# ALRhub/d3il

Measured on AMD Instinct MI355X. Metric: env-steps/s, higher is better.
Workload: dtype f64

## Files before the change

### d3il_amd/capi.py

```python
from __future__ import annotations

import ctypes as C
import os

from .model.blob import ModelBlob

_LIB = None


class Buffers(C.Structure):
    _fields_ = [("n_envs", C.c_int32), ("stride", C.c_int32), ("obs_dim", C.c_int32), ("action_dim", C.c_int32),
                ("obs", C.c_void_p), ("done", C.c_void_p), ("success", C.c_void_p), ("mode", C.c_void_p),
                ("state", C.c_void_p), ("flags", C.c_void_p), ("step_count", C.c_void_p), ("policy_des", C.c_void_p),
                ("info_f64", C.c_void_p), ("n_info_f64", C.c_int32), ("state_rows", C.c_int32), ("last_reset", C.c_void_p)]


STATE_F64 = 42
STATE_QPOS, STATE_QVEL, STATE_BIAS, STATE_TCP, STATE_IK_Q, STATE_IK_QD = 0, 9, 18, 25, 28, 35
FLAG_MODE_MASK, FLAG_TERMINATED, FLAG_SUCCESS, FLAG_ROD_CONTACT = 0x1FF, 1 << 12, 1 << 13, 1 << 14
FLAG_IK_VALID, FLAG_SOLVER_FAIL, FLAG_MULTI_CONTACT = 1 << 15, 1 << 16, 1 << 17
PUSH_STATE_BOX, PUSH_STATE_WARM, PUSH_STATE_TASK, PUSH_STATE_F64 = 42, 68, 89, 91
PFLAG_FIRST_MASK, PFLAG_MODE_MASK, PFLAG_WARM_VALID, PFLAG_CON_OVERFLOW, PFLAG_OFF_TABLE = 0x7, 0x38, 1 << 6, 1 << 18, 1 << 19
PFLAG_LINK_NEAR = 1 << 20
LINK_GUARD_SLACK = 1.25e-4
# ... 28 lines not shown
    if os.environ.get("D3IL_LIB_PATH"):
        return os.environ["D3IL_LIB_PATH"]
    name = "libd3il_rollout_stats.so" if os.environ.get("D3IL_STATS_LIB") == "1" else "libd3il_rollout.so"
    return os.path.join(os.path.dirname(os.path.abspath(__file__)), name)


def load():
    global _LIB
    if _LIB is None:
        path = lib_path()
        if not os.path.exists(path):
            raise D3ilError("%s is missing: build it with `python -m d3il_amd.build` (hipcc, gfx950). "
                            "There is no CPU fallback for the rollout path." % path)
        L = C.CDLL(path)
        L.d3il_last_error.restype = C.c_char_p
        L.d3il_blob_sizeof.restype = C.c_size_t
        L.d3il_create.argtypes = [C.c_int, C.c_int, C.c_int, C.c_void_p, C.c_size_t, C.POINTER(C.c_void_p)]
        L.d3il_destroy.argtypes = [C.c_void_p]
        L.d3il_start.argtypes = [C.c_void_p, C.c_void_p]
        L.d3il_reset.argtypes = [C.c_void_p, C.c_void_p, C.c_void_p, C.c_void_p]
        L.d3il_step.argtypes = [C.c_void_p, C.c_void_p, C.c_void_p]
        L.d3il_get_buffers.argtypes = [C.c_void_p, C.POINTER(Buffers)]
        L.d3il_get_state.argtypes = [C.c_void_p, C.c_void_p, C.c_int32, C.c_void_p, C.c_void_p]
        L.d3il_set_state.argtypes = [C.c_void_p, C.c_void_p, C.c_int32, C.c_void_p, C.c_void_p]
        L.d3il_policy_begin.argtypes = [C.c_void_p, C.c_void_p, C.c_void_p]
        L.d3il_policy_action.argtypes = [C.c_void_p, C.c_uint64, C.c_uint64, C.c_uint32, C.c_void_p, C.c_void_p]
        L.d3il_count_metrics.argtypes = [C.c_void_p, C.c_void_p, C.c_void_p]
        L.d3il_attention_causal_f32.argtypes = [C.c_void_p, C.c_void_p, C.c_int, C.c_int, C.c_int, C.c_int, C.c_void_p]
        L.d3il_layernorm_f32.argtypes = [C.c_void_p, C.c_void_p, C.c_void_p, C.c_void_p, C.c_long, C.c_int, C.c_float, C.c_void_p]
        L.d3il_mlp_ln_gelu_residual_f32.argtypes = [C.c_void_p, C.c_void_p, C.c_void_p, C.c_float, C.c_void_p, C.c_void_p, C.c_void_p, C.c_void_p, C.c_void_p, C.c_long, C.c_int, C.c_int, C.c_void_p]
        L.d3il_linear120_f32.argtypes = [C.c_void_p, C.c_void_p, C.c_void_p, C.c_float, C.c_void_p, C.c_void_p, C.c_void_p, C.c_void_p, C.c_long, C.c_int, C.c_void_p]
        L.d3il_mlp_ln_gelu_residual_f16x3.argtypes = L.d3il_mlp_ln_gelu_residual_f32.argtypes
        L.d3il_linear120_f16x3.argtypes = L.d3il_linear120_f32.argtypes
        L.d3il_attn_half_f16x3.argtypes = [C.c_void_p, C.c_void_p, C.c_void_p, C.c_float, C.c_void_p, C.c_void_p, C.c_void_p, C.c_void_p, C.c_long, C.c_int, C.c_int, C.c_int, C.c_void_p]
        L.d3il_f16x3_set_guard.argtypes = [C.c_void_p]
        L.d3il_bet_head_f32.argtypes = [C.c_void_p, C.c_void_p, C.c_void_p, C.c_float] + [C.c_void_p] * 6 + [C.c_uint64, C.c_uint64] + [C.c_void_p] * 6 + [C.c_long, C.c_int, C.c_int, C.c_int, C.c_void_p]
        L.d3il_ddpm_gpt_step_f32.argtypes = [C.c_void_p, C.c_void_p, C.c_void_p, C.c_float] + [C.c_void_p] * 11 + [C.c_uint64, C.c_uint64] + [C.c_void_p] * 7 + [C.c_long] + [C.c_int] * 5 + [C.c_void_p]
        L.d3il_ibc_langevin_f32.argtypes = [C.c_void_p] * 10 + [C.c_float] + [C.c_void_p] * 5 + [C.c_uint64, C.c_uint64] + [C.c_void_p] * 11 + [C.c_long] + [C.c_int] * 6 + [C.c_void_p]
        L.d3il_act_chunk_f32.argtypes = [C.c_void_p] * 12 + [C.c_uint64, C.c_uint64] + [C.c_void_p] * 6 + [C.c_long] + [C.c_int] * 8 + [C.c_void_p]
        L.d3il_ddpm_act_chunk_f32.argtypes = [C.c_void_p] * 13 + [C.c_uint64, C.c_uint64] + [C.c_void_p] * 9 + [C.c_long] + [C.c_int] * 12 + [C.c_void_p]
        L.d3il_cvae_decode_f32.argtypes = [C.c_void_p] * 11 + [C.c_uint64, C.c_uint64] + [C.c_void_p] * 4 + [C.c_long] + [C.c_int] * 5 + [C.c_void_p]
        L.d3il_ddpm_mlp_f32.argtypes = [C.c_void_p] * 12 + [C.c_long, C.c_int, C.c_int, C.c_int, C.c_int, C.c_void_p]
        L.d3il_resmlp_f32.argtypes = [C.c_void_p] * 8 + [C.c_long, C.c_int, C.c_int, C.c_int, C.c_int, C.c_void_p]
        L.d3il_mlp_gelu_residual_f32.argtypes = [C.c_void_p, C.c_void_p, C.c_void_p, C.c_void_p, C.c_void_p, C.c_void_p, C.c_long, C.c_int, C.c_int, C.c_void_p]
        L.d3il_auto_reset.argtypes = [C.c_void_p, C.c_void_p, C.c_void_p]
        L.d3il_step_auto_reset.argtypes = [C.c_void_p, C.c_void_p, C.c_void_p, C.c_void_p]
        L.d3il_random_rollout_step.argtypes = [C.c_void_p, C.c_uint64, C.c_uint64, C.c_uint32, C.c_void_p, C.c_void_p, C.c_void_p]
        L.d3il_random_rollout_prepare.argtypes = [C.c_void_p, C.c_uint64, C.c_uint64, C.c_uint32, C.c_void_p, C.c_void_p, C.c_void_p]
        L.d3il_timing_stats.argtypes = [C.c_void_p, C.c_void_p]
        L.d3il_set_tally.argtypes = [C.c_void_p, C.c_void_p, C.c_int, C.c_void_p]
        L.d3il_comm_unique_id.argtypes = [C.c_void_p]
        L.d3il_comm_init.argtypes = [C.c_void_p, C.c_int, C.c_int, C.c_int, C.POINTER(C.c_void_p)]
        L.d3il_comm_destroy.argtypes = [C.c_void_p]
        L.d3il_comm_count.argtypes = [C.c_void_p, C.POINTER(C.c_int)]
        L.d3il_rccl_available.restype = C.c_int
        L.d3il_reduce_metrics.argtypes = [C.c_void_p, C.c_void_p, C.c_void_p, C.c_size_t, C.c_void_p]
        L.d3il_set_timing.argtypes = [C.c_void_p, C.c_int]
        L.d3il_last_step_ms.argtypes = [C.c_void_p, C.POINTER(C.c_float)]
        L.d3il_set_option.argtypes = [C.c_void_p, C.c_char_p, C.c_int]
        L.d3il_debug_scratch.argtypes = [C.c_void_p, C.c_int, C.c_void_p, C.c_int]
        L.d3il_debug_build_flags.argtypes = [C.c_void_p]
        L.d3il_set_link_guard.argtypes = [C.c_void_p, C.c_void_p, C.c_int, C.c_double, C.c_void_p]
        if hasattr(L, "d3il_group_create"):
            L.d3il_group_create.argtypes = [C.c_void_p, C.c_int, C.POINTER(C.c_void_p)]
            L.d3il_group_flush.argtypes = [C.c_void_p]
            L.d3il_group_destroy.argtypes = [C.c_void_p]
        if hasattr(L, "d3il_group_set_option"):
            L.d3il_group_set_option.argtypes = [C.c_void_p, C.c_char_p, C.c_int]
            L.d3il_group_stats.argtypes = [C.c_void_p, C.POINTER(C.c_int64), C.POINTER(C.c_int64)]
        if L.d3il_blob_sizeof() != C.sizeof(ModelBlob):
            raise D3ilError("model blob layout mismatch between include/d3il_model_blob.h and d3il_amd/model/blob.py")
        _LIB = L
    return _LIB


def has_step_group() -> bool:
    return hasattr(load(), "d3il_group_create")


def has_group_options() -> bool:
    return hasattr(load(), "d3il_group_set_option")


def check(rc: int):
    if rc != 0:
        raise D3ilError("libd3il_rollout error %d: %s" % (rc, load().d3il_last_error().decode()))


_CAPSULES = os.path.join(os.path.dirname(os.path.abspath(__file__)), "model", "blobs", "panda_link_capsules.json")


def link_capsules(body_names, path: str | None = None):
    import json
    import numpy as np
    with open(path or _CAPSULES) as f:
        js = json.load(f)
    rows = [[body_names.index(c["body"]), c["statics"]] + list(c["p0"]) + list(c["p1"]) + [c["r"]] for c in js["capsules"]]
    return np.ascontiguousarray(rows, dtype=np.float64), float(js["margin"])


def set_link_guard(h, capsules, margin: float, counter_ptr=None):
    import numpy as np
    caps = np.zeros((0, 9)) if capsules is None else np.ascontiguousarray(capsules, dtype=np.float64).reshape(-1, 9)
    check(load().d3il_set_link_guard(h, caps.ctypes.data_as(C.c_void_p) if len(caps) else None, len(caps), float(margin), counter_ptr))
```

### d3il_amd/csrc/rollout.hip

```cpp
#include <hip/hip_runtime.h>
#include <cstdio>
#include <cstdlib>
#include <cstring>
#include <dlfcn.h>
#include <memory>
#include <mutex>
#include <string>
#include "../../include/d3il_rollout.h"
#include "panda_step.h"
#include "rigid_common.h"
#include "gen/avoiding_consts.inc"
#include "gen/stacking_consts.inc"

namespace d3il {
constexpr int WAVE = 64;
}
#include "gen_kernels.h"
#include "link_guard.h"
#include "stack_kernels.h"
#include "policy_f16x3.h"
#include "policy_bet.h"
#include "policy_ddpm_gpt.h"
#include "policy_ibc.h"
#include "policy_act.h"
// ... 871 lines not shown
  if (episode_counts) {
    atomicAdd((unsigned long long*)&episode_counts[0], 1ull);
    if (success[e]) atomicAdd((unsigned long long*)&episode_counts[1], 1ull);
  }
  if (!table) return;
  int c = ctx_id ? ctx_id[e] : 0;
  if (c < 0 || c >= n_ctx) return;
  long long* row = table + (size_t)c * D3IL_TALLY_ROW;
  atomicAdd((unsigned long long*)&row[0], 1ull);
  int code = (int)(short)mode[e] + mode_bias;
  if (success[e]) {
    atomicAdd((unsigned long long*)&row[1], 1ull);
    if (code >= 0 && code < D3IL_TALLY_ROW - 2) atomicAdd((unsigned long long*)&row[2 + code], 1ull);
  }
  if (all_by_code && code >= 0 && code < 256) atomicAdd((unsigned long long*)&row[2 + D3IL_TALLY_ALL + code], 1ull);
}
__global__ void k_store_contexts(const unsigned char* __restrict__ mask, const double* __restrict__ src, double* __restrict__ dst, int n, int dim) {
  int i = blockIdx.x * blockDim.x + threadIdx.x;
  if (i >= n * dim) return;
  if (mask && !mask[i / dim]) return;
  dst[i] = src[i];
}

}

using namespace d3il;

static_assert(D3IL_STACK_STATE_BOX == SK_STATE_BOX && D3IL_STACK_STATE_WARM == SK_STATE_WARM && D3IL_STACK_STATE_F64 == SK_STATE_F64, "d3il_rollout.h: Stacking state layout");
static_assert(D3IL_SFLAG_WARM_VALID == SKF_WARM_VALID && D3IL_SFLAG_HAND_NEAR == SKF_HAND_NEAR && D3IL_PFLAG_CON_OVERFLOW == SKF_CON_OVERFLOW && D3IL_PFLAG_OFF_TABLE == SKF_OFF_TABLE,
              "d3il_rollout.h: Stacking flag bits");
static_assert(D3IL_PFLAG_LINK_NEAR == LG_FLAG && D3IL_PFLAG_LINK_NEAR == D3IL_SFLAG_HAND_NEAR, "d3il_rollout.h: the link-near bit of the generic engine is the hand-near bit of the cooperative one");
static_assert(D3IL_SFLAG_MODE_MASK == (SKF_NMODE_MASK | (0x3Fu << SKF_IND_SHIFT)), "d3il_rollout.h: Stacking order code");
static_assert(D3IL_ALIGN_STATE_BOX == AL_STATE_BOX && D3IL_ALIGN_STATE_WARM == AL_STATE_WARM && D3IL_ALIGN_STATE_TARGET == AL_STATE_TARGET && D3IL_ALIGN_STATE_F64 == AL_STATE_F64, "d3il_rollout.h: Aligning state layout");
static_assert(D3IL_INS_STATE_BOX == 42 && D3IL_INS_STATE_WARM == 42 + 13 * 3 && D3IL_INS_STATE_TASK == 42 + 13 * 3 + 6 * 3 + NDOF && D3IL_INS_STATE_F64 == gen_state_rows(3), "d3il_rollout.h: Inserting state layout");
static_assert(D3IL_PUSH_STATE_BOX == 42 && D3IL_PUSH_STATE_WARM == 42 + 13 * 2 && D3IL_PUSH_STATE_TASK == 42 + 13 * 2 + 6 * 2 + NDOF && D3IL_PUSH_STATE_F64 == gen_state_rows(2) && D3IL_TALLY_ALL + 256 <= D3IL_TALLY_ROW - 2,
              "d3il_rollout.h: Pushing state rows / tally row");

static inline bool gen_task(int task_id) {
  return task_id == D3IL_TASK_SORTING || task_id == D3IL_TASK_INSERTING || task_id == D3IL_TASK_PUSHING;
}

constexpr int RG_SLOTS = 2, RG_SAMPLE = 8;
struct d3il_handle_s {
  int task_id, n, stride, device;
  PandaConsts hc;
  PandaConsts* dc;
  GenConsts gc;
  StackConsts kc;
  AlignTask atk;
  double* d_scratch;
  int state_rows;
  double* d_init_qpos;
  bool started;
  d3il_buffers buf;
  bool fast, timing;
  int split;
  bool serve_avail;
  int serve_max_wg;
  int lanes;
  int lds_pad;
  hipEvent_t ev0, ev1;
  bool ev_valid, ev_created;
  hipEvent_t ring0[128], ring1[128];
  bool ring_created;
  long ring_head, ring_drained, t_n;
  double t_sum, t_min, t_max;
  int tol_mode;
  int stack_reset_coop;
  unsigned long long kc_id;
  double* d_ctx;
  int ctx_dim;
  uint8_t* d_mask;
  const int32_t* tally_ctx; int tally_nctx; int64_t* tally_table;
  bool rg_enabled, rg_ready, rg_capturing, rg_ev_made, rg_timing;
  int rg_slot;
  hipGraph_t rg_graph[RG_SLOTS]; hipGraphExec_t rg_exec[RG_SLOTS];
  unsigned* rg_t_dev; uint32_t rg_next_t; long rg_launched, rg_drained;
  uint64_t rg_seed, rg_off; double* rg_actions; int64_t* rg_counts; hipStream_t rg_stream;
  void* d_reset_img; AvoidResetImage reset_img; AvoidEpilogue* d_epilogue; AvoidEpilogue epilogue_host; bool epilogue_valid; hipStream_t epilogue_stream;
  bool prep_valid; uint32_t prep_t; uint64_t prep_seed, prep_off; double* prep_actions; bool fuse_tail; double* d_des_before; hipStream_t prep_stream;
  bool info_is_view;
  d3il_model_blob model;
  LinkGuardConsts lg; LinkGuardConsts* d_lg; int64_t* lg_flagged;
  struct d3il_group_s* group; bool grp_pending; uint64_t grp_seed, grp_off; uint32_t grp_t; double* grp_actions; int64_t* grp_counts; hipStream_t grp_stream;
  hipEvent_t ring_alt0[128], ring_alt1[128];
};
struct d3il_group_s {
  int device, count; d3il_handle_s* m[AVOID_GROUP_MAX];
  int n_pending; bool busy;
  uint32_t t; int n_substeps, max_steps; bool timing;
  AvoidGroupTable* d_table; AvoidGroupTable table_host; bool table_valid;
  hipEvent_t ev_join[AVOID_GROUP_MAX], ev_done; bool ev_made;
  hipEvent_t ring0[128], ring1[128]; bool ring_created; long ring_head;
  bool quiet, armed; int64_t n_merged, n_joined;
};
static inline void group_arm(d3il_group_s* g) { g->armed = true; }
#if defined(D3IL_EVENT_SYSTEM_FENCE)
constexpr unsigned EV_ORDER_FLAGS = hipEventDisableTiming, EV_TIMING_FLAGS = hipEventDefault;
#else
constexpr unsigned EV_ORDER_FLAGS = hipEventDisableTiming | hipEventDisableSystemFence, EV_TIMING_FLAGS = hipEventDefault | hipEventDisableSystemFence;
#endif

struct ActiveModel { int refs; bool valid; GenConsts gc; StackConsts kc; };
static ActiveModel g_active_gen[16], g_active_stack[16];
static int g_active_tol[16];
static std::mutex g_model_mutex;

static unsigned long long g_stack_loaded_id[16];
static StackConsts g_stack_loaded[16];
static unsigned long long g_kc_counter = 0;

static thread_local std::string g_err;
static int fail(int code, const std::string& msg) { g_err = msg; return code; }
#define HIPCHK(x) do { hipError_t e_ = (x); if (e_ != hipSuccess) return fail(D3IL_EHIP, std::string(#x) + ": " + hipGetErrorString(e_)); } while (0)

extern "C" {

static int group_flush(d3il_group_s* g);
static inline int group_settle(d3il_handle_s* h) {
  if (!h || !h->group || h->group->busy) return D3IL_OK;
  group_arm(h->group);
  return h->group->n_pending ? group_flush(h->group) : D3IL_OK;
}
#define GROUP_SETTLE(h) do { if (int rc_g_ = group_settle(h)) return rc_g_; } while (0)

const char* d3il_last_error(void) { return g_err.c_str(); }
size_t d3il_blob_sizeof(void) { return sizeof(d3il_model_blob); }
int d3il_version(void) { return 2; }

static void rg_drop(d3il_handle_s* h);
static void group_leave(d3il_handle_s* h);
static void rg_drop_for_free(d3il_handle_s* h) {
  if (h->rg_ready) for (int k = 0; k < RG_SLOTS; k++) { (void)hipGraphExecDestroy(h->rg_exec[k]); (void)hipGraphDestroy(h->rg_graph[k]); }
  if (h->rg_t_dev) (void)hipFree(h->rg_t_dev);
}
static void free_handle(d3il_handle_s* h) {
  if (!h) return;
  int dev = h->device;
  if (dev >= 0 && dev < 16) {
    std::lock_guard<std::mutex> lock(g_model_mutex);
    if (gen_task(h->task_id) && g_active_gen[dev].refs > 0) g_active_gen[dev].refs--;
    if (h->task_id == D3IL_TASK_STACKING && g_active_stack[dev].refs > 0) g_active_stack[dev].refs--;
  }
  void* ptrs[] = {h->dc, h->d_init_qpos, h->buf.obs, h->buf.done, h->buf.success, h->buf.mode, h->buf.state, h->buf.flags, h->buf.step_count, h->buf.policy_des,
                  h->info_is_view ? nullptr : (void*)h->buf.info_f64, h->d_scratch, h->d_ctx, h->d_mask, h->d_des_before, h->d_lg, h->d_reset_img, h->d_epilogue};
  for (void* p : ptrs) if (p) (void)hipFree(p);
  if (h->ring_created) for (int i = 0; i < 128; i++) { (void)hipEventDestroy(h->ring0[i]); (void)hipEventDestroy(h->ring1[i]); }
  rg_drop_for_free(h);
  delete h;
}
#define HIPCHK_H(x) do { hipError_t e_ = (x); if (e_ != hipSuccess) { free_handle(h); return fail(D3IL_EHIP, std::string(#x) + ": " + hipGetErrorString(e_)); } } while (0)

int d3il_create(int task_id, int n_envs, int device_id, const void* model_blob, size_t blob_len, d3il_handle* out) {
  if (!out || !model_blob) return fail(D3IL_EINVAL, "d3il_create: null argument");
  *out = nullptr;
  if (blob_len != sizeof(d3il_model_blob)) return fail(D3IL_EBLOB, "d3il_create: blob size mismatch");
  if (n_envs <= 0) return fail(D3IL_EINVAL, "d3il_create: n_envs must be positive");
  const d3il_model_blob& m = *(const d3il_model_blob*)model_blob;
  if (task_id != m.task_id) return fail(D3IL_EINVAL, "d3il_create: task_id does not match the model blob");
  if (task_id != D3IL_TASK_AVOIDING && task_id != D3IL_TASK_PUSHING && task_id != D3IL_TASK_SORTING && task_id != D3IL_TASK_STACKING && task_id != D3IL_TASK_ALIGNING && task_id != D3IL_TASK_INSERTING)
    return fail(D3IL_EUNSUPPORTED, "d3il_create: unknown task id (Avoiding, Pushing, Sorting, Stacking, Aligning and Inserting are implemented)");
  int ndev = 0;
  if (hipGetDeviceCount(&ndev) != hipSuccess || ndev <= 0) return fail(D3IL_ENODEVICE, "d3il_create: no HIP device available (there is no CPU fallback)");
  if (device_id < 0 || device_id >= ndev || device_id >= 16) return fail(D3IL_ENODEVICE, "d3il_create: device_id out of range");
  HIPCHK(hipSetDevice(device_id));
  d3il_handle_s* h = new d3il_handle_s();
  std::memset(&h->buf, 0, sizeof h->buf);
  h->task_id = -1; h->device = device_id;
  h->model = m; h->d_lg = nullptr; h->lg_flagged = nullptr; h->lg.n = 0;
  h->dc = nullptr; h->d_init_qpos = nullptr; h->d_scratch = nullptr; h->d_ctx = nullptr; h->d_mask = nullptr; h->ev_created = false; h->ring_created = false;
  h->tally_ctx = nullptr; h->tally_nctx = 0; h->tally_table = nullptr; h->tol_mode = 0; h->ctx_dim = 0; h->stack_reset_coop = 1; h->kc_id = 0;
  const char* err = "";
  int rc = build_panda_consts(m, h->hc, &err);
  if (rc) { free_handle(h); return fail(D3IL_EBLOB, std::string("d3il_create: ") + err); }
  finish_invweights(h->hc);
  if (gen_task(task_id) && build_gen_consts(m, h->hc, h->gc, &err)) { free_handle(h); return fail(D3IL_EBLOB, std::string("d3il_create: ") + err); }
  if (task_id == D3IL_TASK_STACKING && build_stack_consts(m, h->hc, h->kc, &err)) { free_handle(h); return fail(D3IL_EBLOB, std::string("d3il_create: ") + err); }
  if (task_id == D3IL_TASK_ALIGNING && build_coop_align_consts(m, h->hc, h->kc, h->atk, &err)) { free_handle(h); return fail(D3IL_EBLOB, std::string("d3il_create: ") + err); }
  {
// ... 862 lines not shown
  if (!(h->rg_enabled && h->task_id == D3IL_TASK_AVOIDING && stream != nullptr && h->started)) return D3IL_OK;
  hipStream_t s = (hipStream_t)stream;
  HIPCHK(hipSetDevice(h->device));
  if (h->rg_ready && (h->rg_seed != seed || h->rg_off != env_offset || h->rg_actions != actions || h->rg_counts != episode_counts_device || h->rg_stream != s ||
                      h->rg_timing != h->timing)) {
    HIPCHK(hipStreamSynchronize(h->rg_stream));
    rg_drop(h);
  }
  if (!h->rg_ready) return rg_capture(h, seed, env_offset, t, actions, episode_counts_device, s);
  return D3IL_OK;
}
static bool continues_sequence(const d3il_handle_s* h, uint64_t seed, uint64_t env_offset, uint32_t t, const double* actions, void* stream) {
  return h->prep_valid && h->prep_t == t && h->prep_seed == seed && h->prep_off == env_offset && h->prep_actions == actions && h->prep_stream == (hipStream_t)stream;
}
static int fused_step_begin(d3il_handle h, uint64_t seed, uint64_t env_offset, uint32_t t, double* actions, int64_t* episode_counts_device, void* stream, AvoidEpilogue& a) {
  const bool cont = continues_sequence(h, seed, env_offset, t, actions, stream);
  if (!h->d_des_before) { HIPCHK(hipSetDevice(h->device)); HIPCHK(hipMalloc(&h->d_des_before, (size_t)h->stride * 2 * sizeof(double))); }
  if (cont) h->prep_valid = 0;
  else { if (int rc = d3il_policy_action(h, seed, env_offset, t, actions, stream)) return rc; }
  d3il_buffers& b = h->buf;
  a = AvoidEpilogue{};
  a.img = h->reset_img; a.state = b.state; a.flags = b.flags; a.steps = b.step_count; a.obs = b.obs; a.done = b.done; a.success = b.success; a.mode = b.mode;
  a.n = h->n; a.stride = h->stride; a.des = b.policy_des; a.episode_counts = (long long*)episode_counts_device; a.mask = h->d_mask; a.ctx_id = h->tally_ctx;
  a.table = (long long*)h->tally_table; a.actions = actions; a.des_before = h->d_des_before; a.seed = seed; a.env_offset = env_offset; a.n_ctx = h->tally_nctx;
  if (split_step_kernel(h)) {
    if (!h->epilogue_valid || std::memcmp(&h->epilogue_host, &a, sizeof a) != 0) {
      HIPCHK(hipSetDevice(h->device));
      if (h->epilogue_valid && (h->epilogue_stream != (hipStream_t)stream || h->group)) HIPCHK(hipDeviceSynchronize());
      HIPCHK(hipMemcpyAsync(h->d_epilogue, &a, sizeof a, hipMemcpyHostToDevice, (hipStream_t)stream));
      HIPCHK(hipStreamSynchronize((hipStream_t)stream));
      h->epilogue_host = a; h->epilogue_valid = true; h->epilogue_stream = (hipStream_t)stream;
    }
  }
  return D3IL_OK;
}
static void fused_step_end(d3il_handle h, uint64_t seed, uint64_t env_offset, uint32_t t, double* actions, void* stream) {
  h->prep_valid = true; h->prep_t = t + 1u; h->prep_seed = seed; h->prep_off = env_offset; h->prep_actions = actions; h->prep_stream = (hipStream_t)stream;
}
static int rollout_step_single(d3il_handle h, uint64_t seed, uint64_t env_offset, uint32_t t, double* actions, int64_t* episode_counts_device, void* stream) {
  if (h && h->rg_enabled && h->task_id == D3IL_TASK_AVOIDING && stream != nullptr && actions && h->started) {
    hipStream_t s = (hipStream_t)stream;
    if (int rc_ = drop_prepared_action(h)) return rc_;
    if (int rc = d3il_random_rollout_prepare(h, seed, env_offset, t, actions, episode_counts_device, stream)) return rc;
    if (t != h->rg_next_t) { HIPCHK(hipMemcpyAsync(h->rg_t_dev, &t, sizeof(unsigned), hipMemcpyHostToDevice, s)); HIPCHK(hipStreamSynchronize(s)); }
    if (h->timing && h->rg_launched % RG_SAMPLE == RG_SAMPLE - 1) {
      if (int rc = d3il_policy_action(h, seed, env_offset, t, actions, stream)) return rc;
      if (int rc = d3il_step(h, actions, stream)) return rc;
      if (int rc = d3il_auto_reset(h, episode_counts_device, stream)) return rc;
      hipLaunchKernelGGL(k_inc_counter, dim3(1), dim3(64), 0, s, h->rg_t_dev);
      HIPCHK(hipGetLastError());
    } else HIPCHK(hipGraphLaunch(h->rg_exec[h->rg_launched % RG_SLOTS], s));
    h->rg_launched++; h->rg_next_t = t + 1;
    return D3IL_OK;
  }
  if (h && h->fuse_tail && h->task_id == D3IL_TASK_AVOIDING && actions && episode_counts_device && h->started) {
    AvoidEpilogue a;
    if (int rc = fused_step_begin(h, seed, env_offset, t, actions, episode_counts_device, stream, a)) return rc;
    if (split_step_kernel(h)) {
      if (int rc = step_launch(h, actions, stream, h->d_epilogue, t + 1u)) return rc;
    } else {
      if (int rc = d3il_step(h, actions, stream)) return rc;
      hipLaunchKernelGGL(k_avoiding_tail, dim3(h->stride / WAVE), dim3(WAVE), 0, (hipStream_t)stream, a, t + 1u);
      HIPCHK(hipGetLastError());
    }
    fused_step_end(h, seed, env_offset, t, actions, stream);
    return D3IL_OK;
  }
  if (int rc = d3il_policy_action(h, seed, env_offset, t, actions, stream)) return rc;
  if (int rc = d3il_step(h, actions, stream)) return rc;
  return d3il_auto_reset(h, episode_counts_device, stream);
}

static int group_flush(d3il_group_s* g) {
  if (g->busy) return D3IL_OK;
  group_arm(g);
  g->busy = true;
  int rc = D3IL_OK;
  for (int i = 0; i < g->count; i++) {
    d3il_handle_s* h = g->m[i];
    if (!h->grp_pending) continue;
    h->grp_pending = false; g->n_pending--;
    if (!rc) rc = rollout_step_single(h, h->grp_seed, h->grp_off, h->grp_t, h->grp_actions, h->grp_counts, (void*)h->grp_stream);
  }
  g->n_pending = 0; g->busy = false;
  return rc;
}
static int group_launch_locked(d3il_group_s* g) {
  HIPCHK(hipSetDevice(g->device));
  if (!g->ev_made) {
    for (int i = 0; i < AVOID_GROUP_MAX; i++) HIPCHK(hipEventCreateWithFlags(&g->ev_join[i], EV_ORDER_FLAGS));
    HIPCHK(hipEventCreateWithFlags(&g->ev_done, EV_ORDER_FLAGS));
    HIPCHK(hipMalloc(&g->d_table, sizeof(AvoidGroupTable)));
    g->ev_made = true;
  }
  AvoidGroupTable tab;
  std::memset(&tab, 0, sizeof tab);
  unsigned total = 0; int serve_budget = 0;
  for (int i = 0; i < AVOID_GROUP_MAX; i++) tab.m[i].first_wg = 0xFFFFFFFFu;
  for (int i = 0; i < g->count; i++) {
    d3il_handle_s* h = g->m[i];
    AvoidEpilogue a;
    if (int rc = fused_step_begin(h, h->grp_seed, h->grp_off, h->grp_t, h->grp_actions, h->grp_counts, (void*)h->grp_stream, a)) return rc;
    const d3il_buffers& b = h->buf;
    AvoidGroupMember& r = tab.m[i];
    r.state = b.state; r.flags = b.flags; r.steps = b.step_count; r.actions = h->grp_actions; r.obs = b.obs; r.done = b.done; r.success = b.success; r.mode = b.mode;
    r.ep = h->d_epilogue; r.n = h->n; r.stride = h->stride; r.first_wg = total;
    total += (unsigned)((h->n + WAVE - 1) / WAVE); serve_budget += h->serve_max_wg;
  }
  hipStream_t s0 = g->m[0]->grp_stream;
  if (!g->table_valid || std::memcmp(&g->table_host, &tab, sizeof tab) != 0) {
    if (g->table_valid) HIPCHK(hipDeviceSynchronize());
    HIPCHK(hipMemcpy(g->d_table, &tab, sizeof tab, hipMemcpyHostToDevice));
    g->table_host = tab; g->table_valid = true;
  }
  const bool join = !g->quiet || g->armed;
  if (join) for (int i = 1; i < g->count; i++) {
    if (g->m[i]->grp_stream == s0) continue;
    HIPCHK(hipEventRecord(g->ev_join[i], g->m[i]->grp_stream));
    HIPCHK(hipStreamWaitEvent(s0, g->ev_join[i], 0));
  }
  hipEvent_t t0 = nullptr, t1 = nullptr;
  if (g->timing) {
    if (!g->ring_created) {
      for (int i = 0; i < 128; i++) { HIPCHK(hipEventCreateWithFlags(&g->ring0[i], EV_TIMING_FLAGS)); HIPCHK(hipEventCreateWithFlags(&g->ring1[i], EV_TIMING_FLAGS)); }
      g->ring_created = true;
    }
    for (int i = 0; i < g->count; i++) { d3il_handle_s* h = g->m[i]; if (h->ring_head - h->ring_drained >= 128) { if (int rc = timing_drain_one(h)) return rc; } }
    t0 = g->ring0[g->ring_head % 128]; t1 = g->ring1[g->ring_head % 128];
    HIPCHK(hipEventRecord(t0, s0));
  }
  const d3il_handle_s* h0 = g->m[0];
  const unsigned t_next = g->t + 1u;
  if ((long)total <= (long)serve_budget)
    hipLaunchKernelGGL((k_avoiding_step_split<true, true, true>), dim3(total), dim3(3 * WAVE), AVOID_LDS_SERVE, s0, (const AvoidGroupTable*)g->d_table, (double*)nullptr, (unsigned*)nullptr,
                       (int*)nullptr, (const double*)nullptr, (float*)nullptr, (unsigned char*)nullptr, (unsigned char*)nullptr, (unsigned short*)nullptr, 0, 0, h0->hc.n_substeps,
                       h0->hc.max_steps, (const AvoidEpilogue*)nullptr, t_next);
  else
    hipLaunchKernelGGL((k_avoiding_step_split<true, false, true>), dim3(total), dim3(2 * WAVE), 0, s0, (const AvoidGroupTable*)g->d_table, (double*)nullptr, (unsigned*)nullptr,
                       (int*)nullptr, (const double*)nullptr, (float*)nullptr, (unsigned char*)nullptr, (unsigned char*)nullptr, (unsigned short*)nullptr, 0, 0, h0->hc.n_substeps,
                       h0->hc.max_steps, (const AvoidEpilogue*)nullptr, t_next);
  HIPCHK(hipGetLastError());
  hipEvent_t done_ev = g->ev_done;
  if (g->timing) {
    HIPCHK(hipEventRecord(t1, s0));
    done_ev = t1;
    for (int i = 0; i < g->count; i++) {
      d3il_handle_s* h = g->m[i];
      const int slot = (int)(h->ring_head % 128);
      h->ring_alt0[slot] = t0; h->ring_alt1[slot] = t1; h->ev0 = t0; h->ev1 = t1; h->ev_valid = true; h->ring_head++;
    }
    g->ring_head++;
  } else HIPCHK(hipEventRecord(done_ev, s0));
  for (int i = 1; i < g->count; i++) if (g->m[i]->grp_stream != s0) HIPCHK(hipStreamWaitEvent(g->m[i]->grp_stream, done_ev, 0));
  for (int i = 0; i < g->count; i++) { d3il_handle_s* h = g->m[i]; fused_step_end(h, h->grp_seed, h->grp_off, h->grp_t, h->grp_actions, (void*)h->grp_stream); }
  g->n_merged++; g->n_joined += join ? 1 : 0;
  g->armed = false;
  return D3IL_OK;
}
static int group_launch(d3il_group_s* g) {
  g->busy = true;
  const int rc = group_launch_locked(g);
  if (rc) group_arm(g);
  for (int i = 0; i < g->count; i++) g->m[i]->grp_pending = false;
  g->n_pending = 0; g->busy = false;
  return rc;
}
static int group_rollout_step(d3il_handle h, uint64_t seed, uint64_t env_offset, uint32_t t, double* actions, int64_t* episode_counts_device, void* stream, int* handled) {
  d3il_group_s* g = h->group;
  *handled = 0;
  if (g->busy) return D3IL_OK;
  const bool eligible = h->fuse_tail && !h->rg_enabled && h->task_id == D3IL_TASK_AVOIDING && actions && episode_counts_device && h->started && split_step_kernel(h) &&
                        h->serve_avail && continues_sequence(h, seed, env_offset, t, actions, stream);
  if (!eligible) {
    group_arm(g);
    return g->n_pending ? group_flush(g) : D3IL_OK;
  }
  if (g->n_pending && (h->grp_pending || g->t != t || g->n_substeps != h->hc.n_substeps || g->max_steps != h->hc.max_steps || g->timing != h->timing)) {
    if (int rc = group_flush(g)) return rc;
  }
  if (!g->n_pending) { g->t = t; g->n_substeps = h->hc.n_substeps; g->max_steps = h->hc.max_steps; g->timing = h->timing; }
  h->grp_pending = true; h->grp_seed = seed; h->grp_off = env_offset; h->grp_t = t; h->grp_actions = actions; h->grp_counts = episode_counts_device; h->grp_stream = (hipStream_t)stream;
  g->n_pending++;
  *handled = 1;
  return g->n_pending == g->count ? group_launch(g) : D3IL_OK;
}
int d3il_random_rollout_step(d3il_handle h, uint64_t seed, uint64_t env_offset, uint32_t t, double* actions, int64_t* episode_counts_device, void* stream) {
  if (h && h->group) {
    int handled = 0;
    if (int rc = group_rollout_step(h, seed, env_offset, t, actions, episode_counts_device, stream, &handled)) return rc;
    if (handled) return D3IL_OK;
  }
  return rollout_step_single(h, seed, env_offset, t, actions, episode_counts_device, stream);
}
static void timing_drain_all(d3il_handle_s* h) { while (h->ring_drained < h->ring_head) { if (timing_drain_one(h)) { h->ring_drained = h->ring_head; break; } } }
static void group_leave(d3il_handle_s* h) {
  d3il_group_s* g = h->group;
  if (!g) return;
  (void)group_flush(g);
  group_arm(g);
  timing_drain_all(h);
  if (h->ring_head > 0 && h->ring_alt0[(h->ring_head - 1) % 128]) { h->ev_valid = false; h->ev0 = h->ev1 = nullptr; }
  for (int i = 0; i < 128; i++) h->ring_alt0[i] = h->ring_alt1[i] = nullptr;
  int k = 0;
  for (int i = 0; i < g->count; i++) if (g->m[i] != h) g->m[k++] = g->m[i];
  g->count = k; h->group = nullptr; h->grp_pending = false;
}
int d3il_group_create(const d3il_handle* handles, int count, d3il_group* out) {
  if (!handles || !out) return fail(D3IL_EINVAL, "d3il_group_create: null argument");
  *out = nullptr;
  if (count < 1 || count > AVOID_GROUP_MAX) return fail(D3IL_EINVAL, "d3il_group_create: a group has 1 .. 8 members");
  for (int i = 0; i < count; i++) {
    d3il_handle_s* h = handles[i];
    if (!h) return fail(D3IL_EINVAL, "d3il_group_create: null handle");
    if (h->task_id != D3IL_TASK_AVOIDING) return fail(D3IL_EUNSUPPORTED, "d3il_group_create: Avoiding handles only");
    if (h->device != handles[0]->device) return fail(D3IL_EINVAL, "d3il_group_create: the members must live on one device");
    if (h->group) return fail(D3IL_ESTATE, "d3il_group_create: a handle is already in a group");
    for (int j = 0; j < i; j++) if (handles[j] == h) return fail(D3IL_EINVAL, "d3il_group_create: a handle is listed twice");
  }
  HIPCHK(hipSetDevice(handles[0]->device));
  if (hipFuncSetAttribute((const void*)k_avoiding_step_split<true, true, true>, hipFuncAttributeMaxDynamicSharedMemorySize, (int)AVOID_LDS_SERVE) != hipSuccess) (void)hipGetLastError();
  d3il_group_s* g = new d3il_group_s();
  g->device = handles[0]->device; g->count = count;
  g->armed = true;
  for (int i = 0; i < count; i++) { g->m[i] = handles[i]; handles[i]->group = g; handles[i]->grp_pending = false; }
  *out = g;
  return D3IL_OK;
}
int d3il_group_flush(d3il_group g) {
  if (!g) return fail(D3IL_EINVAL, "d3il_group_flush: null group");
  group_arm(g);
  return g->n_pending ? group_flush(g) : D3IL_OK;
}
int d3il_group_set_option(d3il_group g, const char* name, int value) {
  if (!g || !name) return fail(D3IL_EINVAL, "d3il_group_set_option: null argument");
  if (std::strcmp(name, "quiet_streams") == 0) {
    if (value != 0 && value != 1) return fail(D3IL_EINVAL, "quiet_streams must be 0 or 1");
    group_arm(g);
    if (g->n_pending) { if (int rc = group_flush(g)) return rc; }
    g->quiet = value != 0;
    return D3IL_OK;
  }
  return fail(D3IL_EINVAL, std::string("d3il_group_set_option: unknown option ") + name);
}
int d3il_group_stats(d3il_group g, int64_t* merged_rounds, int64_t* joined_rounds) {
  if (!g || !merged_rounds || !joined_rounds) return fail(D3IL_EINVAL, "d3il_group_stats: null argument");
  *merged_rounds = g->n_merged; *joined_rounds = g->n_joined;
  return D3IL_OK;
}
int d3il_group_destroy(d3il_group g) {
  if (!g) return fail(D3IL_EINVAL, "d3il_group_destroy: null group");
  (void)hipSetDevice(g->device);
  const int rc = group_flush(g);
  while (g->count > 0) group_leave(g->m[g->count - 1]);
  (void)hipDeviceSynchronize();
  if (g->ev_made) { for (int i = 0; i < AVOID_GROUP_MAX; i++) (void)hipEventDestroy(g->ev_join[i]); (void)hipEventDestroy(g->ev_done); (void)hipFree(g->d_table); }
  if (g->ring_created) for (int i = 0; i < 128; i++) { (void)hipEventDestroy(g->ring0[i]); (void)hipEventDestroy(g->ring1[i]); }
  delete g;
  return rc;
}
int d3il_last_step_ms(d3il_handle h, float* ms) {
  GROUP_SETTLE(h);
  if (!h || !ms) return fail(D3IL_EINVAL, "d3il_last_step_ms: null argument");
  if (!h->ev_valid) return fail(D3IL_ESTATE, "d3il_last_step_ms: timing not enabled or no step recorded");
  HIPCHK(hipEventSynchronize(h->ev1));
  HIPCHK(hipEventElapsedTime(ms, h->ev0, h->ev1));
  return D3IL_OK;
}
int d3il_debug_wave_stats(uint64_t* out, int nwaves, int reset) {
#if defined(D3IL_DEVICE_STATS)
  HIPCHK(hipDeviceSynchronize());
  HIPCHK(hipMemcpyFromSymbol(out, HIP_SYMBOL(d3il::g_dev_wave), (size_t)nwaves * 10 * sizeof(unsigned long long)));
  if (reset) { static unsigned long long z[4096][10]; HIPCHK(hipMemcpyToSymbol(HIP_SYMBOL(d3il::g_dev_wave), z, sizeof z)); }
  return D3IL_OK;
#else
  (void)out; (void)nwaves; (void)reset;
  return fail(D3IL_EUNSUPPORTED, "d3il_debug_wave_stats: library built without D3IL_DEVICE_STATS");
#endif
}

int d3il_debug_wave_counts(uint64_t* out, int nwaves, int reset) {
#if defined(D3IL_DEVICE_STATS)
  HIPCHK(hipDeviceSynchronize());
  HIPCHK(hipMemcpyFromSymbol(out, HIP_SYMBOL(d3il::g_dev_cnt), (size_t)nwaves * 8 * sizeof(unsigned long long)));
  if (reset) { static unsigned long long z[4096][8]; HIPCHK(hipMemcpyToSymbol(HIP_SYMBOL(d3il::g_dev_cnt), z, sizeof z)); }
  return D3IL_OK;
#else
  (void)out; (void)nwaves; (void)reset;
  return fail(D3IL_EUNSUPPORTED, "d3il_debug_wave_counts: library built without D3IL_DEVICE_STATS");
#endif
}

int d3il_debug_stats(uint64_t* out32, int reset) {
#if defined(D3IL_DEVICE_STATS)
  unsigned long long tmp[32];
  HIPCHK(hipDeviceSynchronize());
  HIPCHK(hipMemcpyFromSymbol(tmp, HIP_SYMBOL(d3il::g_dev_stats), sizeof tmp));
  for (int i = 0; i < 32; i++) out32[i] = tmp[i];
  if (reset) { unsigned long long z[32] = {0}; HIPCHK(hipMemcpyToSymbol(HIP_SYMBOL(d3il::g_dev_stats), z, sizeof z)); }
  return D3IL_OK;
#else
  (void)out32; (void)reset;
  return fail(D3IL_EUNSUPPORTED, "d3il_debug_stats: library built without D3IL_DEVICE_STATS");
#endif
}

int d3il_debug_scratch(d3il_handle h, int env, double* out, int count) {
  GROUP_SETTLE(h);
  if (!h || !out) return fail(D3IL_EINVAL, "d3il_debug_scratch: null argument");
  if (!h->d_scratch || env < 0 || env >= h->n) return fail(D3IL_EINVAL, "d3il_debug_scratch: no scratch area / env out of range");
  HIPCHK(hipSetDevice(h->device));
  HIPCHK(hipDeviceSynchronize());
  if (h->task_id == D3IL_TASK_STACKING || h->task_id == D3IL_TASK_ALIGNING) {
    if (count > SG_SIZE) return fail(D3IL_EINVAL, "d3il_debug_scratch: count exceeds the environment's scratch area");
    HIPCHK(hipMemcpy(out, h->d_scratch + (size_t)env * SG_SIZE, (size_t)count * sizeof(double), hipMemcpyDeviceToHost));
    return D3IL_OK;
  }
  if (gen_task(h->task_id)) {
    if (count > GG_SIZE) return fail(D3IL_EINVAL, "d3il_debug_scratch: count exceeds the environment's scratch area");
    const double* base = h->d_scratch + (size_t)(env / GEN_LANES) * GG_BLOCK * GEN_LANES + 2 * (env % GEN_LANES);
    HIPCHK(hipMemcpy2D(out, 2 * sizeof(double), base, (size_t)2 * GEN_LANES * sizeof(double), sizeof(double), (size_t)(count + 1) / 2, hipMemcpyDeviceToHost));
    HIPCHK(hipMemcpy2D(out + 1, 2 * sizeof(double), base + 1, (size_t)2 * GEN_LANES * sizeof(double), sizeof(double), (size_t)count / 2, hipMemcpyDeviceToHost));
    return D3IL_OK;
  }
  HIPCHK(hipMemcpy2D(out, sizeof(double), h->d_scratch + env, (size_t)h->stride * sizeof(double), sizeof(double), (size_t)count, hipMemcpyDeviceToHost));
  return D3IL_OK;
}

int d3il_debug_build_flags(int* out8) {
  if (!out8) return fail(D3IL_EINVAL, "d3il_debug_build_flags: null argument");
  int f = 0;
#if defined(D3IL_POISON)
  f |= D3IL_BUILD_POISON;
#endif
#if defined(D3IL_SK_POISON)
  f |= D3IL_BUILD_SK_POISON;
#endif
#if defined(D3IL_DEVICE_STATS)
  f |= D3IL_BUILD_STATS;
#endif
// ... 39 lines not shown
```

### d3il_amd/envs/avoiding.py

```python
from __future__ import annotations

import ctypes as C

import numpy as np
import torch

from .. import capi
from ..controllers.offline_ik import offline_ik
from ..kinematics import UrdfChain
from ..model import blob as blob_mod


class _DevArray:

    def __init__(self, ptr, shape, typestr, owner):
        self.__cuda_array_interface__ = {"shape": tuple(shape), "typestr": typestr, "data": (int(ptr), False), "version": 2}
        self._owner = owner


def _view(ptr, shape, typestr, device, owner):
    return torch.as_tensor(_DevArray(ptr, shape, typestr, owner), device=device)


class StepGroup:

    MAX_MEMBERS = 8

    def __init__(self, envs, quiet_streams: bool = False):
        envs = list(envs)
        if not capi.has_step_group():
            raise capi.D3ilError("the loaded libd3il_rollout has no step group (d3il_group_create)")
        self.L = capi.load()
        arr = (C.c_void_p * len(envs))(*[e.h for e in envs])
        g = C.c_void_p()
        capi.check(self.L.d3il_group_create(arr, len(envs), C.byref(g)))
        self.g = g
        if quiet_streams:
            self.set_option("quiet_streams", 1)

    def set_option(self, name: str, value: int):
        if not capi.has_group_options():
            raise capi.D3ilError("the loaded libd3il_rollout has no group options (d3il_group_set_option)")
        capi.check(self.L.d3il_group_set_option(self.g, name.encode(), int(value)))

    def stats(self):
        merged, joined = C.c_int64(), C.c_int64()
        capi.check(self.L.d3il_group_stats(self.g, C.byref(merged), C.byref(joined)))
        return merged.value, joined.value

    def flush(self):
        if self.g:
            capi.check(self.L.d3il_group_flush(self.g))

    def close(self):
        if getattr(self, "g", None):
            self.L.d3il_group_destroy(self.g)
            self.g = None

    def __del__(self):
        try:
            self.close()
        except Exception:
            pass


class ObstacleAvoidanceVecEnv:
    task = "avoiding"
    action_dim = 7
    obs_dim = 2

    default_max_steps = 250

    def __init__(self, n_envs: int, device: int | str | torch.device = 0, render: bool = False,
                 n_substeps: int = 35, max_steps_per_episode: int | None = None):
        if max_steps_per_episode is None:
            max_steps_per_episode = self.default_max_steps
        if render:
            raise NotImplementedError("rendering is outside the batched rollout path")
        dev = torch.device(device if not isinstance(device, int) else "cuda:%d" % device)
        if dev.type != "cuda":
            raise capi.D3ilError("%s needs a HIP device (got %s); there is no CPU fallback" % (type(self).__name__, dev))
        self.device = dev
        self.n_envs = int(n_envs)
        self.L = capi.load()
        self.js = blob_mod.load_json(self.task)
        self.js["task_const"]["n_substeps"] = int(n_substeps)
        self.js["task_const"]["max_steps"] = int(max_steps_per_episode)
        self.blob = blob_mod.pack(self.js)
        self.n_substeps, self.max_steps_per_episode = int(n_substeps), int(max_steps_per_episode)
        h = C.c_void_p()
        capi.check(self.L.d3il_create(self.blob.task_id, self.n_envs, dev.index or 0, C.byref(self.blob), C.sizeof(self.blob), C.byref(h)))
        self.h = h
        b = capi.Buffers()
        capi.check(self.L.d3il_get_buffers(self.h, C.byref(b)))
        self.stride = b.stride
        n, s = self.n_envs, b.stride
        self.obs = _view(b.obs, (n, b.obs_dim), "<f4", dev, self)
        self.done = _view(b.done, (n,), "|u1", dev, self)
        self.success = _view(b.success, (n,), "|u1", dev, self)
        self.mode = _view(b.mode, (n,), "<i2", dev, self)
        self.state_rows = b.state_rows
        self.state = _view(b.state, (b.state_rows, s), "<f8", dev, self)
        self.info_f64 = _view(b.info_f64, (b.n_info_f64, s), "<f8", dev, self) if b.n_info_f64 else None
        self.flags = _view(b.flags, (s,), "<i4", dev, self)
        self.step_count = _view(b.step_count, (s,), "<i4", dev, self)
        self.policy_des = _view(b.policy_des, (3, s), "<f8", dev, self)
        self.last_reset = _view(b.last_reset, (n,), "|u1", dev, self)
        self._tally = None
        self._bound_stream = None
        self.init_qpos = None
        self._started = False

    def start(self):
        c, tc = self.js["controller"], self.js["task_const"]
        chain = UrdfChain(self.js["urdf_chain"])
        target = list(tc["init_end_eff_pos"]) + list(tc["init_end_eff_quat"])
        q, iters, err = offline_ik(chain, c["default_qpos"], target, np.array(c["joint_pos_min"]), np.array(c["joint_pos_max"]))
        self.set_init_qpos(q)
        return q, iters, err

    def set_init_qpos(self, q):
        q = np.ascontiguousarray(q, dtype=np.float64)
        capi.check(self.L.d3il_start(self.h, q.ctypes.data_as(C.c_void_p)))
        self.init_qpos = q.copy()
        self._started = True

# ... 126 lines not shown
```

### d3il_amd/envs/sub_batch.py

```python
from __future__ import annotations

import copy
import os
import warnings

import torch

MIN_ENVS = 64
DEFAULT_HW_QUEUES = 4
MAX_CONCURRENT = 4
CUS = 256


def plan(n: int, n_sub_batches: int, min_envs: int = MIN_ENVS):
    s = max(1, min(int(n_sub_batches), n // min_envs if n >= min_envs else 1))
    base, extra = divmod(n, s)
    out, off = [], 0
    for i in range(s):
        c = base + (1 if i < extra else 0)
        out.append((off, c))
        off += c
    return out


def ensure_hw_queues(n_streams: int):
    cur = os.environ.get("GPU_MAX_HW_QUEUES")
    have = int(cur) if cur and cur.isdigit() else DEFAULT_HW_QUEUES
    if have >= n_streams:
        return have
    if not torch.cuda.is_initialized():
        os.environ["GPU_MAX_HW_QUEUES"] = str(n_streams)
        return n_streams
    warnings.warn("%d sub-batches but GPU_MAX_HW_QUEUES = %d was fixed when HIP initialised: their streams share hardware queues and will not fully "
                  "overlap (export GPU_MAX_HW_QUEUES=%d before the first GPU call)" % (n_streams, have, n_streams))
    return have


def fork_agent(agent):
    if hasattr(agent, "fork"):
        return agent.fork()
    from ..agents import _is_lane_state
    c = copy.copy(agent)
    for k, v in list(vars(agent).items()):
        if k.startswith("_parameters") or k.startswith("_modules") or k.startswith("_buffers"):
            continue
        if _is_lane_state(v):
            setattr(c, k, copy.deepcopy(v))
    return c


class SubBatch:
    __slots__ = ("index", "offset", "n", "env", "stream", "own_stream", "agent", "state")

    def __init__(self, index, offset, n, env, stream, own_stream):
        self.index, self.offset, self.n, self.env, self.stream, self.own_stream = index, offset, n, env, stream, own_stream
        self.agent, self.state = None, None


class SubBatchSet:

    def __init__(self, n: int, n_sub_batches: int, device, make_env, min_envs: int = MIN_ENVS):
        self.device = torch.device(device)
        self.parts = plan(n, n_sub_batches, min_envs)
        self.n = n
        S = len(self.parts)
        hw_queues = ensure_hw_queues(S) if S > 1 else DEFAULT_HW_QUEUES
        self.group = None
        if S > MAX_CONCURRENT:
            warnings.warn("%d sub-batches: the GPU runs %d dispatches of different streams at a time, the others wait their turn (DESIGN section 19.6)" % (S, MAX_CONCURRENT))
        self.default_stream = torch.cuda.current_stream(self.device)
        self.batches = []
        for i, (off, cnt) in enumerate(self.parts):
            own = S > 1
            stream = torch.cuda.Stream(self.device) if own else self.default_stream
            with torch.cuda.stream(stream):
                env = make_env(cnt, off)
                if own:
                    env.bind_stream(stream)
                if own and hasattr(env, "set_option") and type(env).__name__ == "ObstacleAvoidanceVecEnv":
                    env.set_option("serve_wave_max_workgroups", CUS // S)
            self.batches.append(SubBatch(i, off, cnt, env, stream, own))
        if S > 1:
            for b in self.batches:
                self.default_stream.wait_stream(b.stream)
            self.group = self._step_group(hw_queues)

    def _step_group(self, hw_queues: int):
        envs = [b.env for b in self.batches]
        want = hw_queues < len(envs) + 1
        if os.environ.get("D3IL_STEP_GROUP") in ("0", "1"):
            want = os.environ["D3IL_STEP_GROUP"] == "1"
        if not want or not all(type(e).__name__ == "ObstacleAvoidanceVecEnv" for e in envs):
            return None
        from .avoiding import StepGroup
        from .. import capi
        if len(envs) > StepGroup.MAX_MEMBERS or not capi.has_step_group():
            return None
        return StepGroup(envs, quiet_streams=capi.has_group_options())

    def __len__(self):
        return len(self.batches)

    def __iter__(self):
        return iter(self.batches)

    def each(self, fn):
        if len(self.batches) == 1:
            fn(self.batches[0])
            return
        try:
            for b in self.batches:
                torch.cuda.set_stream(b.stream)
                fn(b)
        finally:
            torch.cuda.set_stream(self.default_stream)

    def join(self):
        if self.group is not None:
            self.group.flush()
        if len(self.batches) > 1:
            for b in self.batches:
                self.default_stream.wait_stream(b.stream)

    def fork_agents(self, agent):
        from ..agents import as_batched
        for b in self.batches:
            a = agent if len(self.batches) == 1 else fork_agent(agent)
            if hasattr(a, "set_rollout_range"):
                a.set_rollout_range(b.offset, b.n)
            b.agent = as_batched(a, b.n)
            if b.agent is not a and hasattr(b.agent, "set_rollout_range"):
                b.agent.set_rollout_range(b.offset, b.n)
            b.agent.reset()

    @property
    def link_near_episodes(self) -> int:
        return sum(int(getattr(b.env, "link_near_episodes", 0)) for b in self.batches if b.env is not None)

    def close(self):
        if self.group is not None:
            self.group.close()
            self.group = None
        for b in self.batches:
            if b.env is not None:
                b.env.close()
                b.env = None
```

Baseline: 7.094 million.

## Split avoiding step group into multiple independent dispatch sets

Adds dispatch sets to the step group so the member envs can be split into subsets. Each subset launches its own merged fused step with its own events and table, instead of waiting for every member. The Python side picks two sets when there are at least four members, the member count is even and at least three hardware queues exist. This is meant to overlap merged dispatches across hardware queues and cut join latency, at the cost of more launches and per-set event bookkeeping.

```diff
diff --git a/d3il_amd/capi.py b/d3il_amd/capi.py
--- a/d3il_amd/capi.py
+++ b/d3il_amd/capi.py
@@ -134,6 +134,10 @@
     return hasattr(load(), "d3il_group_set_option")
 
 
+def is_unknown_group_option(err: Exception) -> bool:
+    return isinstance(err, D3ilError) and "d3il_group_set_option: unknown option" in str(err)
+
+
 def check(rc: int):
     if rc != 0:
         raise D3ilError("libd3il_rollout error %d: %s" % (rc, load().d3il_last_error().decode()))
diff --git a/d3il_amd/csrc/rollout.hip b/d3il_amd/csrc/rollout.hip
--- a/d3il_amd/csrc/rollout.hip
+++ b/d3il_amd/csrc/rollout.hip
@@ -977,19 +977,25 @@
   bool info_is_view;
   d3il_model_blob model;
   LinkGuardConsts lg; LinkGuardConsts* d_lg; int64_t* lg_flagged;
-  struct d3il_group_s* group; bool grp_pending; uint64_t grp_seed, grp_off; uint32_t grp_t; double* grp_actions; int64_t* grp_counts; hipStream_t grp_stream;
+  struct d3il_group_s* group; int grp_set; bool grp_pending; uint64_t grp_seed, grp_off; uint32_t grp_t; double* grp_actions; int64_t* grp_counts; hipStream_t grp_stream;
   hipEvent_t ring_alt0[128], ring_alt1[128];
 };
-struct d3il_group_s {
-  int device, count; d3il_handle_s* m[AVOID_GROUP_MAX];
-  int n_pending; bool busy;
+struct d3il_dispatch_set {
+  int count; d3il_handle_s* m[AVOID_GROUP_MAX];
+  int n_pending;
   uint32_t t; int n_substeps, max_steps; bool timing;
   AvoidGroupTable* d_table; AvoidGroupTable table_host; bool table_valid;
   hipEvent_t ev_join[AVOID_GROUP_MAX], ev_done; bool ev_made;
   hipEvent_t ring0[128], ring1[128]; bool ring_created; long ring_head;
-  bool quiet, armed; int64_t n_merged, n_joined;
+  bool armed;
 };
-static inline void group_arm(d3il_group_s* g) { g->armed = true; }
+struct d3il_group_s {
+  int device, count; d3il_handle_s* m[AVOID_GROUP_MAX];
+  int n_sets; d3il_dispatch_set set[AVOID_GROUP_MAX];
+  int n_pending; bool busy;
+  bool quiet; int64_t n_merged, n_joined;
+};
+static inline void group_arm(d3il_group_s* g) { for (int k = 0; k < AVOID_GROUP_MAX; k++) g->set[k].armed = true; }
 #if defined(D3IL_EVENT_SYSTEM_FENCE)
 constexpr unsigned EV_ORDER_FLAGS = hipEventDisableTiming, EV_TIMING_FLAGS = hipEventDefault;
 #else
@@ -2018,11 +2024,12 @@
     h->grp_pending = false; g->n_pending--;
     if (!rc) rc = rollout_step_single(h, h->grp_seed, h->grp_off, h->grp_t, h->grp_actions, h->grp_counts, (void*)h->grp_stream);
   }
+  for (int k = 0; k < g->n_sets; k++) g->set[k].n_pending = 0;
   g->n_pending = 0; g->busy = false;
   return rc;
 }
-static int group_launch_locked(d3il_group_s* g) {
-  HIPCHK(hipSetDevice(g->device));
+static int group_launch_locked(d3il_group_s* grp, d3il_dispatch_set* g) {
+  HIPCHK(hipSetDevice(grp->device));
   if (!g->ev_made) {
     for (int i = 0; i < AVOID_GROUP_MAX; i++) HIPCHK(hipEventCreateWithFlags(&g->ev_join[i], EV_ORDER_FLAGS));
     HIPCHK(hipEventCreateWithFlags(&g->ev_done, EV_ORDER_FLAGS));
@@ -2049,7 +2056,7 @@
     HIPCHK(hipMemcpy(g->d_table, &tab, sizeof tab, hipMemcpyHostToDevice));
     g->table_host = tab; g->table_valid = true;
   }
-  const bool join = !g->quiet || g->armed;
+  const bool join = !grp->quiet || g->armed;
   if (join) for (int i = 1; i < g->count; i++) {
     if (g->m[i]->grp_stream == s0) continue;
     HIPCHK(hipEventRecord(g->ev_join[i], g->m[i]->grp_stream));
@@ -2089,16 +2096,22 @@
   } else HIPCHK(hipEventRecord(done_ev, s0));
   for (int i = 1; i < g->count; i++) if (g->m[i]->grp_stream != s0) HIPCHK(hipStreamWaitEvent(g->m[i]->grp_stream, done_ev, 0));
   for (int i = 0; i < g->count; i++) { d3il_handle_s* h = g->m[i]; fused_step_end(h, h->grp_seed, h->grp_off, h->grp_t, h->grp_actions, (void*)h->grp_stream); }
-  g->n_merged++; g->n_joined += join ? 1 : 0;
+  grp->n_merged++; grp->n_joined += join ? 1 : 0;
   g->armed = false;
   return D3IL_OK;
 }
-static int group_launch(d3il_group_s* g) {
+static int group_launch(d3il_group_s* g, d3il_dispatch_set* s) {
   g->busy = true;
-  const int rc = group_launch_locked(g);
-  if (rc) group_arm(g);
-  for (int i = 0; i < g->count; i++) g->m[i]->grp_pending = false;
-  g->n_pending = 0; g->busy = false;
+  const int rc = group_launch_locked(g, s);
+  for (int i = 0; i < s->count; i++) s->m[i]->grp_pending = false;
+  g->n_pending -= s->n_pending; s->n_pending = 0;
+  if (rc) {
+    group_arm(g);
+    for (int i = 0; i < g->count; i++) g->m[i]->grp_pending = false;
+    for (int k = 0; k < g->n_sets; k++) g->set[k].n_pending = 0;
+    g->n_pending = 0;
+  }
+  g->busy = false;
   return rc;
 }
 static int group_rollout_step(d3il_handle h, uint64_t seed, uint64_t env_offset, uint32_t t, double* actions, int64_t* episode_counts_device, void* stream, int* handled) {
@@ -2111,14 +2124,15 @@
     group_arm(g);
     return g->n_pending ? group_flush(g) : D3IL_OK;
   }
-  if (g->n_pending && (h->grp_pending || g->t != t || g->n_substeps != h->hc.n_substeps || g->max_steps != h->hc.max_steps || g->timing != h->timing)) {
+  d3il_dispatch_set* s = &g->set[h->grp_set];
+  if (s->n_pending && (h->grp_pending || s->t != t || s->n_substeps != h->hc.n_substeps || s->max_steps != h->hc.max_steps || s->timing != h->timing)) {
     if (int rc = group_flush(g)) return rc;
   }
-  if (!g->n_pending) { g->t = t; g->n_substeps = h->hc.n_substeps; g->max_steps = h->hc.max_steps; g->timing = h->timing; }
+  if (!s->n_pending) { s->t = t; s->n_substeps = h->hc.n_substeps; s->max_steps = h->hc.max_steps; s->timing = h->timing; }
   h->grp_pending = true; h->grp_seed = seed; h->grp_off = env_offset; h->grp_t = t; h->grp_actions = actions; h->grp_counts = episode_counts_device; h->grp_stream = (hipStream_t)stream;
-  g->n_pending++;
+  s->n_pending++; g->n_pending++;
   *handled = 1;
-  return g->n_pending == g->count ? group_launch(g) : D3IL_OK;
+  return s->n_pending == s->count ? group_launch(g, s) : D3IL_OK;
 }
 int d3il_random_rollout_step(d3il_handle h, uint64_t seed, uint64_t env_offset, uint32_t t, double* actions, int64_t* episode_counts_device, void* stream) {
   if (h && h->group) {
@@ -2129,17 +2143,40 @@
   return rollout_step_single(h, seed, env_offset, t, actions, episode_counts_device, stream);
 }
 static void timing_drain_all(d3il_handle_s* h) { while (h->ring_drained < h->ring_head) { if (timing_drain_one(h)) { h->ring_drained = h->ring_head; break; } } }
+static void group_forget_events(d3il_handle_s* h) {
+  timing_drain_all(h);
+  if (h->ring_head > 0 && h->ring_alt0[(h->ring_head - 1) % 128]) { h->ev_valid = false; h->ev0 = h->ev1 = nullptr; }
+  for (int i = 0; i < 128; i++) h->ring_alt0[i] = h->ring_alt1[i] = nullptr;
+}
 static void group_leave(d3il_handle_s* h) {
   d3il_group_s* g = h->group;
   if (!g) return;
   (void)group_flush(g);
   group_arm(g);
-  timing_drain_all(h);
-  if (h->ring_head > 0 && h->ring_alt0[(h->ring_head - 1) % 128]) { h->ev_valid = false; h->ev0 = h->ev1 = nullptr; }
-  for (int i = 0; i < 128; i++) h->ring_alt0[i] = h->ring_alt1[i] = nullptr;
+  group_forget_events(h);
+  d3il_dispatch_set* s = &g->set[h->grp_set];
+  if (h->grp_pending) { s->n_pending--; g->n_pending--; }
   int k = 0;
+  for (int i = 0; i < s->count; i++) if (s->m[i] != h) s->m[k++] = s->m[i];
+  s->count = k;
+  k = 0;
   for (int i = 0; i < g->count; i++) if (g->m[i] != h) g->m[k++] = g->m[i];
   g->count = k; h->group = nullptr; h->grp_pending = false;
+}
+static void group_partition(d3il_group_s* g, int k) {
+  const int base = g->count / k, extra = g->count % k;
+  g->n_sets = k;
+  int i = 0;
+  for (int j = 0; j < AVOID_GROUP_MAX; j++) {
+    d3il_dispatch_set* s = &g->set[j];
+    s->count = j < k ? base + (j < extra ? 1 : 0) : 0;
+    s->n_pending = 0;
+    for (int q = 0; q < s->count; q++, i++) {
+      d3il_handle_s* h = g->m[i];
+      if (h->grp_set != j) group_forget_events(h);
+      s->m[q] = h; h->grp_set = j;
+    }
+  }
 }
 int d3il_group_create(const d3il_handle* handles, int count, d3il_group* out) {
   if (!handles || !out) return fail(D3IL_EINVAL, "d3il_group_create: null argument");
@@ -2157,8 +2194,9 @@
   if (hipFuncSetAttribute((const void*)k_avoiding_step_split<true, true, true>, hipFuncAttributeMaxDynamicSharedMemorySize, (int)AVOID_LDS_SERVE) != hipSuccess) (void)hipGetLastError();
   d3il_group_s* g = new d3il_group_s();
   g->device = handles[0]->device; g->count = count;
-  g->armed = true;
-  for (int i = 0; i < count; i++) { g->m[i] = handles[i]; handles[i]->group = g; handles[i]->grp_pending = false; }
+  group_arm(g);
+  for (int i = 0; i < count; i++) { g->m[i] = handles[i]; handles[i]->group = g; handles[i]->grp_set = 0; handles[i]->grp_pending = false; }
+  group_partition(g, 1);
   *out = g;
   return D3IL_OK;
 }
@@ -2176,6 +2214,14 @@
     g->quiet = value != 0;
     return D3IL_OK;
   }
+  if (std::strcmp(name, "dispatch_sets") == 0) {
+    if (value < 1 || value > g->count) return fail(D3IL_EINVAL, "dispatch_sets must be 1 .. the number of members");
+    group_arm(g);
+    if (g->n_pending) { if (int rc = group_flush(g)) return rc; }
+    (void)hipSetDevice(g->device);
+    group_partition(g, value);
+    return D3IL_OK;
+  }
   return fail(D3IL_EINVAL, std::string("d3il_group_set_option: unknown option ") + name);
 }
 int d3il_group_stats(d3il_group g, int64_t* merged_rounds, int64_t* joined_rounds) {
@@ -2189,8 +2235,11 @@
   const int rc = group_flush(g);
   while (g->count > 0) group_leave(g->m[g->count - 1]);
   (void)hipDeviceSynchronize();
-  if (g->ev_made) { for (int i = 0; i < AVOID_GROUP_MAX; i++) (void)hipEventDestroy(g->ev_join[i]); (void)hipEventDestroy(g->ev_done); (void)hipFree(g->d_table); }
-  if (g->ring_created) for (int i = 0; i < 128; i++) { (void)hipEventDestroy(g->ring0[i]); (void)hipEventDestroy(g->ring1[i]); }
+  for (int k = 0; k < AVOID_GROUP_MAX; k++) {
+    d3il_dispatch_set* s = &g->set[k];
+    if (s->ev_made) { for (int i = 0; i < AVOID_GROUP_MAX; i++) (void)hipEventDestroy(s->ev_join[i]); (void)hipEventDestroy(s->ev_done); (void)hipFree(s->d_table); }
+    if (s->ring_created) for (int i = 0; i < 128; i++) { (void)hipEventDestroy(s->ring0[i]); (void)hipEventDestroy(s->ring1[i]); }
+  }
   delete g;
   return rc;
 }
diff --git a/d3il_amd/envs/avoiding.py b/d3il_amd/envs/avoiding.py
--- a/d3il_amd/envs/avoiding.py
+++ b/d3il_amd/envs/avoiding.py
@@ -26,7 +26,7 @@
 
     MAX_MEMBERS = 8
 
-    def __init__(self, envs, quiet_streams: bool = False):
+    def __init__(self, envs, quiet_streams: bool = False, dispatch_sets: int = 1):
         envs = list(envs)
         if not capi.has_step_group():
             raise capi.D3ilError("the loaded libd3il_rollout has no step group (d3il_group_create)")
@@ -37,11 +37,27 @@
         self.g = g
         if quiet_streams:
             self.set_option("quiet_streams", 1)
+        self.dispatch_sets = 1
+        if dispatch_sets != 1:
+            self.set_option("dispatch_sets", dispatch_sets)
 
     def set_option(self, name: str, value: int):
         if not capi.has_group_options():
             raise capi.D3ilError("the loaded libd3il_rollout has no group options (d3il_group_set_option)")
         capi.check(self.L.d3il_group_set_option(self.g, name.encode(), int(value)))
+        if name == "dispatch_sets":
+            self.dispatch_sets = int(value)
+
+    def try_option(self, name: str, value: int) -> bool:
+        if not capi.has_group_options():
+            return False
+        try:
+            self.set_option(name, value)
+        except capi.D3ilError as e:
+            if capi.is_unknown_group_option(e):
+                return False
+            raise
+        return True
 
     def stats(self):
         merged, joined = C.c_int64(), C.c_int64()
diff --git a/d3il_amd/envs/sub_batch.py b/d3il_amd/envs/sub_batch.py
--- a/d3il_amd/envs/sub_batch.py
+++ b/d3il_amd/envs/sub_batch.py
@@ -96,7 +96,13 @@
         from .. import capi
         if len(envs) > StepGroup.MAX_MEMBERS or not capi.has_step_group():
             return None
-        return StepGroup(envs, quiet_streams=capi.has_group_options())
+        group = StepGroup(envs, quiet_streams=capi.has_group_options())
+        sets = 2 if len(envs) >= 4 and len(envs) % 2 == 0 and hw_queues >= 3 else 1
+        if os.environ.get("D3IL_STEP_GROUP_SETS") in ("1", "2"):
+            sets = int(os.environ["D3IL_STEP_GROUP_SETS"])
+        if sets != 1 and sets <= len(envs):
+            group.try_option("dispatch_sets", sets)
+        return group
 
     def __len__(self):
         return len(self.batches)
```

Result: faster. 7.478 million, median of 6 (+5.4%).
